# AI4Science-WestlakeU/safediffcon

Hardware: AMD Instinct MI355X
Metric: sampled control trajectories/sec (1000-step DDPM) (higher is better)
Workload: dtype f32; 1 GPU; C4: 2D smoke Unet3D_with_Conv3D dim=64 (1,2,4) state (B,32,7,64,64), B=64 per GPU, guided 1000-step DDPM, conformal quantile on; batch_per_gpu=64, global_batch=64, step=U-Net + guidance + posterior update of the whole batch, one hipGraph replay, parallelism=batch-sharded x1, no data-path collective, conv_precision=fp32

## Files before the change

include/sdc.h:

```cpp
#ifndef SDC_H
#define SDC_H

#include <stddef.h>
#include <stdint.h>

#ifdef __cplusplus
extern "C" {
#endif

#define SDC_OK 0
#define SDC_EINVAL (-1)
#define SDC_EALIGN (-2)
#define SDC_EHIP (-3)
#define SDC_ENULL (-4)

int sdc_version(void);
int sdc_last_error(char* buf, size_t cap);

typedef struct SdcConvDesc {
    int32_t B, Cin0, Cin1, Cout;
    int32_t iD, iH, iW;
    int32_t oD, oH, oW;
    int32_t kD, kH, kW;
    int32_t sD, sH, sW;
// ... 33 lines not shown
int sdc_gn_pointwise_out(const float* h, const float* stats, const float* gamma, const float* beta, const float* residual,
                         const float* w, const float* bias, float* y, int B, int C, int G, int Cout, int64_t S, int64_t plane,
                         int64_t ys0, int64_t ys1, int64_t ys2, void* stream);

int sdc_chan_norm(const float* x, const float* g, const float* residual, float* y, int B, int C, int64_t S,
                  int mode, float eps, void* stream);

int sdc_linattn(const float* qkv, float* ctx, float* out, int outer, int inner, int heads, int64_t n,
                int64_t q_so, int64_t q_sc, int64_t q_si, int64_t o_so, int64_t o_sc, int64_t o_si, void* stream);

size_t sdc_linattn_block_bytes(int outer, int inner, int C, int64_t n);
int sdc_linattn_block(const float* x, const float* g_pre, const float* wqkv, const float* wo, const float* bo,
                      const float* g_post, float* work, float* y, int outer, int inner, int C, int64_t n,
                      int64_t so, int64_t sc, int64_t si, int pre_mode, int post_mode, float eps, void* stream);
int sdc_linattn_block_gn(const float* x_raw, const float* gn_stats, const float* gn_gamma, const float* gn_beta, int gn_G,
                         const float* gn_residual, const float* g_pre, const float* wqkv, const float* wo, const float* bo,
                         const float* g_post, float* work, float* y, int outer, int inner, int C, int64_t n,
                         int64_t so, int64_t sc, int64_t si, int pre_mode, int post_mode, float eps, void* stream);
int sdc_linattn_block_sel(const float* x, const float* g_pre, const float* wqkv, const float* wo, const float* bo,
                          const float* g_post, float* work, float* y, int outer, int inner, int C, int64_t n,
                          int64_t so, int64_t sc, int64_t si, int pre_mode, int post_mode, float eps, int impl, void* stream);
int sdc_linattn_block_gn_sel(const float* x_raw, const float* gn_stats, const float* gn_gamma, const float* gn_beta, int gn_G,
                             const float* gn_residual, const float* g_pre, const float* wqkv, const float* wo, const float* bo,
                             const float* g_post, float* work, float* y, int outer, int inner, int C, int64_t n,
                             int64_t so, int64_t sc, int64_t si, int pre_mode, int post_mode, float eps, int impl, void* stream);
int sdc_linattn_block_x3_ok(int C, int64_t n);

size_t sdc_pack_linattn_f16_bytes(int C);
int sdc_pack_linattn_f16(const float* wqkv, const float* wo, int C, void* dst, void* stream);
size_t sdc_linattn_block_f16_bytes(int outer, int inner, int C, int64_t n);
int sdc_linattn_block_f16(const float* x, const float* g_pre, const float* wqkv, const float* wo, const void* wpk, const float* bo,
                          const float* g_post, void* work, float* y, int outer, int inner, int C, int64_t n,
                          int64_t so, int64_t sc, int64_t si, int pre_mode, int post_mode, float eps, void* stream);
int sdc_linattn_block_gn_f16(const float* x_raw, const float* gn_stats, const float* gn_gamma, const float* gn_beta, int gn_G,
                             const float* gn_residual, const float* g_pre, const float* wqkv, const float* wo, const void* wpk,
                             const float* bo, const float* g_post, void* work, float* y, int outer, int inner, int C, int64_t n,
                             int64_t so, int64_t sc, int64_t si, int pre_mode, int post_mode, float eps, void* stream);
int sdc_linattn_block_f16_ok(int C, int64_t n);

int sdc_tattn_block(const float* x, const float* g_pre, const float* wqkv, const float* wo, const float* rot,
                    const float* bias, float* y, int outer, int inner, int C, int ntok, int64_t so, int64_t sc,
                    int64_t st, float eps, void* stream);

size_t sdc_pack_tattn_f16_bytes(void);
int sdc_pack_tattn_f16(const float* wqkv, const float* wo, void* dst, void* stream);
int sdc_tattn_block_f16(const float* x, const float* g_pre, const void* wpk, const float* rot, const float* bias, float* y,
                        int outer, int inner, int C, int ntok, int64_t so, int64_t sc, int64_t st, float eps, void* stream);

size_t sdc_pack_tattn_x3_bytes(void);
int sdc_pack_tattn_x3(const float* wqkv, const float* wo, void* dst, void* stream);
int sdc_tattn_block_x3(const float* x, const float* g_pre, const void* wpk, const float* rot, const float* bias, float* y,
                       int outer, int inner, int C, int ntok, int64_t so, int64_t sc, int64_t st, float eps, void* stream);
int sdc_tattn_block_x3_ok(int C, int ntok, int inner);

int sdc_attn(const float* qkv, float* out, const float* rot, const float* bias, int outer, int inner, int heads,
             int ntok, int64_t q_so, int64_t q_sc, int64_t q_si, int64_t q_st,
             int64_t o_so, int64_t o_sc, int64_t o_si, int64_t o_st, void* stream);

int sdc_act(const float* x, float* y, int64_t n, int kind, void* stream);

#define SDC_MODEL_BURGERS 0
#define SDC_MODEL_TOKAMAK 1
#define SDC_MODEL_SMOKE 2

typedef struct SdcStepDesc {
    int32_t model;
    int32_t B;
    int32_t d0, d1, d2, d3;
    int32_t guide;
    int32_t clip;
    int32_t impose;
    int32_t cond_idx;
    int32_t pad_zero;
    int32_t use_max;
    int32_t has_wgt;
    int32_t skip_draws;
    int32_t ddim;
    uint64_t seed;
} SdcStepDesc;

int sdc_guide_reduce(const SdcStepDesc* d, const float* x, const float* eps, const float* coef, const int32_t* t_dev,
                     const float* gpar, float* gscal, void* stream);
int sdc_step_update(const SdcStepDesc* d, const float* x, const float* eps, const float* gext, const float* coef,
                    const int32_t* t_dev, const int32_t* draw_dev, const float* noise, int64_t noise_stride,
                    const float* gpar, const float* gscal, const float* target, const float* c0, const float* c1,
                    const float* c2, float* xout, float* x0out, void* stream);
int sdc_impose(const SdcStepDesc* d, float* x, const float* c0, const float* c1, const float* c2, void* stream);
int sdc_randn(float* x, int64_t n, uint64_t seed, const int32_t* draw_dev, void* stream);
int sdc_advance(int32_t* t_dev, int dt, int32_t* draw_dev, int ddraw, void* stream);

int sdc_advance_table(int32_t* idx_dev, int32_t* t_dev, const int32_t* ttab, int32_t* draw_dev, int ddraw, void* stream);

int sdc_conformal_score(const SdcStepDesc* d, const float* pred, const float* truth, const float* target,
                        const float* gpar, float* score, float* weight, void* stream);

int sdc_burgers_rollout(const float* u0, const float* f, float* traj, int N, int s, int Nt, int steps, int record_every,
                        float dt, float coef_transport, float d0, float d1, float d2, void* stream);


typedef struct SdcWgradDesc {
    int32_t B, M, N;
    int32_t oD, oH, oW;
    int32_t iD, iH, iW;
    int32_t kD, kH, kW;
    int32_t sD, sH, sW;
    int32_t pD, pH, pW;
// ... 187 lines not shown
```

safediffcon_amd/_lib.py:

```python
import ctypes as C
import os

_HERE = os.path.dirname(os.path.abspath(__file__))
LIB_PATH = os.path.join(_HERE, "libsdc_hip.so")

SDC_MODEL_BURGERS, SDC_MODEL_TOKAMAK, SDC_MODEL_SMOKE = 0, 1, 2

_f32p = C.c_void_p
_i32p = C.c_void_p
_stream = C.c_void_p
_i64 = C.c_int64


class SdcConvDesc(C.Structure):
    _fields_ = [(n, C.c_int32) for n in (
        "B", "Cin0", "Cin1", "Cout", "iD", "iH", "iW", "oD", "oH", "oW", "kD", "kH", "kW", "sD", "sH", "sW",
        "pD", "pH", "pW", "uD", "uH", "uW", "up_mode", "precision")] + [
        ("x0s", C.c_int64 * 5), ("x1s", C.c_int64 * 5), ("ys", C.c_int64 * 5), ("rs", C.c_int64 * 5)]


class SdcStepDesc(C.Structure):
    _fields_ = [(n, C.c_int32) for n in (
        "model", "B", "d0", "d1", "d2", "d3", "guide", "clip", "impose", "cond_idx", "pad_zero", "use_max",
        "has_wgt", "skip_draws", "ddim")] + [("_pad", C.c_int32), ("seed", C.c_uint64)]
# ... 36 lines not shown
                ("low_action", C.c_double * 9), ("high_action", C.c_double * 9), ("year_in", C.c_double)]


SIGNATURES = {
    "sdc_version": (C.c_int, []),
    "sdc_last_error": (C.c_int, [C.c_char_p, C.c_size_t]),
    "sdc_conv": (C.c_int, [C.POINTER(SdcConvDesc), _f32p, _f32p, _f32p, _f32p, _f32p, _f32p, _stream]),
    "sdc_conv_describe": (C.c_int, [C.POINTER(SdcConvDesc), C.c_char_p, C.c_size_t, C.POINTER(C.c_double)]),
    "sdc_conv_gnparts": (C.c_int, [C.POINTER(SdcConvDesc), C.c_int]),
    "sdc_conv_gn": (C.c_int, [C.POINTER(SdcConvDesc), _f32p, _f32p, _f32p, _f32p, _f32p, _f32p, C.c_void_p, C.c_int, _stream]),
    "sdc_gn_finalize": (C.c_int, [C.c_void_p, _f32p, C.c_int, C.c_int, C.c_int, _i64, C.c_float, _stream]),
    "sdc_gn_stats": (C.c_int, [_f32p, _f32p, C.c_int, C.c_int, C.c_int, _i64, C.c_float, _stream]),
    "sdc_gn_stats_bytes": (C.c_size_t, [C.c_int, C.c_int]),
    "sdc_gn_apply": (C.c_int, [_f32p, _f32p, _f32p, _f32p, _f32p, _i32p, _i64, _i64, _i64, _f32p, _f32p,
                               C.c_int, C.c_int, C.c_int, _i64, _stream]),
    "sdc_gn_fused_ok": (C.c_int, [C.c_int, C.c_int, C.c_int, _i64]),
    "sdc_gn_fused": (C.c_int, [_f32p, _f32p, _f32p, _f32p, _i32p, _i64, _i64, _i64, _f32p, _f32p, C.c_int, C.c_int, C.c_int, _i64,
                               C.c_float, _stream]),
    "sdc_gn_pointwise_out": (C.c_int, [_f32p, _f32p, _f32p, _f32p, _f32p, _f32p, _f32p, _f32p, C.c_int, C.c_int, C.c_int, C.c_int, _i64,
                                       _i64, _i64, _i64, _i64, _stream]),
    "sdc_chan_norm": (C.c_int, [_f32p, _f32p, _f32p, _f32p, C.c_int, C.c_int, _i64, C.c_int, C.c_float, _stream]),
    "sdc_linattn": (C.c_int, [_f32p, _f32p, _f32p, C.c_int, C.c_int, C.c_int, _i64, _i64, _i64, _i64, _i64, _i64,
                              _i64, _stream]),
    "sdc_linattn_block_bytes": (C.c_size_t, [C.c_int, C.c_int, C.c_int, _i64]),
    "sdc_linattn_block": (C.c_int, [_f32p, _f32p, _f32p, _f32p, _f32p, _f32p, _f32p, _f32p, C.c_int, C.c_int, C.c_int, _i64,
                                    _i64, _i64, _i64, C.c_int, C.c_int, C.c_float, _stream]),
    "sdc_linattn_block_gn": (C.c_int, [_f32p, _f32p, _f32p, _f32p, C.c_int, _f32p, _f32p, _f32p, _f32p, _f32p, _f32p, _f32p, _f32p,
                                       C.c_int, C.c_int, C.c_int, _i64, _i64, _i64, _i64, C.c_int, C.c_int, C.c_float, _stream]),
    "sdc_linattn_block_sel": (C.c_int, [_f32p, _f32p, _f32p, _f32p, _f32p, _f32p, _f32p, _f32p, C.c_int, C.c_int, C.c_int, _i64,
                                        _i64, _i64, _i64, C.c_int, C.c_int, C.c_float, C.c_int, _stream]),
    "sdc_linattn_block_gn_sel": (C.c_int, [_f32p, _f32p, _f32p, _f32p, C.c_int, _f32p, _f32p, _f32p, _f32p, _f32p, _f32p, _f32p, _f32p,
                                           C.c_int, C.c_int, C.c_int, _i64, _i64, _i64, _i64, C.c_int, C.c_int, C.c_float, C.c_int, _stream]),
    "sdc_linattn_block_x3_ok": (C.c_int, [C.c_int, _i64]),
    "sdc_pack_linattn_f16_bytes": (C.c_size_t, [C.c_int]),
    "sdc_pack_linattn_f16": (C.c_int, [_f32p, _f32p, C.c_int, C.c_void_p, _stream]),
    "sdc_linattn_block_f16_bytes": (C.c_size_t, [C.c_int, C.c_int, C.c_int, _i64]),
    "sdc_linattn_block_f16": (C.c_int, [_f32p, _f32p, _f32p, _f32p, C.c_void_p, _f32p, _f32p, C.c_void_p, _f32p, C.c_int, C.c_int,
                                        C.c_int, _i64, _i64, _i64, _i64, C.c_int, C.c_int, C.c_float, _stream]),
    "sdc_linattn_block_gn_f16": (C.c_int, [_f32p, _f32p, _f32p, _f32p, C.c_int, _f32p, _f32p, _f32p, _f32p, C.c_void_p, _f32p, _f32p,
                                           C.c_void_p, _f32p, C.c_int, C.c_int, C.c_int, _i64, _i64, _i64, _i64, C.c_int, C.c_int,
                                           C.c_float, _stream]),
    "sdc_linattn_block_f16_ok": (C.c_int, [C.c_int, _i64]),
    "sdc_tattn_block": (C.c_int, [_f32p, _f32p, _f32p, _f32p, _f32p, _f32p, _f32p, C.c_int, C.c_int, C.c_int, C.c_int,
                                  _i64, _i64, _i64, C.c_float, _stream]),
    "sdc_pack_tattn_f16_bytes": (C.c_size_t, []),
    "sdc_pack_tattn_f16": (C.c_int, [_f32p, _f32p, C.c_void_p, _stream]),
    "sdc_tattn_block_f16": (C.c_int, [_f32p, _f32p, C.c_void_p, _f32p, _f32p, _f32p, C.c_int, C.c_int, C.c_int, C.c_int,
                                      _i64, _i64, _i64, C.c_float, _stream]),
    "sdc_pack_tattn_x3_bytes": (C.c_size_t, []),
    "sdc_pack_tattn_x3": (C.c_int, [_f32p, _f32p, C.c_void_p, _stream]),
    "sdc_tattn_block_x3": (C.c_int, [_f32p, _f32p, C.c_void_p, _f32p, _f32p, _f32p, C.c_int, C.c_int, C.c_int, C.c_int,
                                     _i64, _i64, _i64, C.c_float, _stream]),
    "sdc_tattn_block_x3_ok": (C.c_int, [C.c_int, C.c_int, C.c_int]),
    "sdc_attn": (C.c_int, [_f32p, _f32p, _f32p, _f32p, C.c_int, C.c_int, C.c_int, C.c_int, _i64, _i64, _i64, _i64,
                           _i64, _i64, _i64, _i64, _stream]),
    "sdc_act": (C.c_int, [_f32p, _f32p, _i64, C.c_int, _stream]),
    "sdc_guide_reduce": (C.c_int, [C.POINTER(SdcStepDesc), _f32p, _f32p, _f32p, _i32p, _f32p, _f32p, _stream]),
    "sdc_step_update": (C.c_int, [C.POINTER(SdcStepDesc), _f32p, _f32p, _f32p, _f32p, _i32p, _i32p, _f32p, _i64,
                                  _f32p, _f32p, _f32p, _f32p, _f32p, _f32p, _f32p, _f32p, _stream]),
    "sdc_impose": (C.c_int, [C.POINTER(SdcStepDesc), _f32p, _f32p, _f32p, _f32p, _stream]),
    "sdc_randn": (C.c_int, [_f32p, _i64, C.c_uint64, _i32p, _stream]),
    "sdc_advance": (C.c_int, [_i32p, C.c_int, _i32p, C.c_int, _stream]),
    "sdc_advance_table": (C.c_int, [_i32p, _i32p, _i32p, _i32p, C.c_int, _stream]),
    "sdc_conformal_score": (C.c_int, [C.POINTER(SdcStepDesc), _f32p, _f32p, _f32p, _f32p, _f32p, _f32p, _stream]),
    "sdc_burgers_rollout": (C.c_int, [_f32p, _f32p, _f32p, C.c_int, C.c_int, C.c_int, C.c_int, C.c_int, C.c_float, C.c_float,
                                      C.c_float, C.c_float, C.c_float, _stream]),
    "sdc_conv_wgrad_bytes": (C.c_size_t, [C.POINTER(SdcWgradDesc)]),
    "sdc_conv_wgrad": (C.c_int, [C.POINTER(SdcWgradDesc), _f32p, _f32p, _f32p, _f32p, C.c_void_p, C.c_size_t, _stream]),
    "sdc_f16_grad_exponent": (C.c_int, [_f32p, C.c_int, C.c_int, C.c_int, C.c_int, C.c_int, C.c_void_p, C.c_void_p, _stream]),
    "sdc_conv_dgrad_f16": (C.c_int, [C.POINTER(SdcConvDesc), _f32p, _f32p, C.c_void_p, _f32p, _stream]),
    "sdc_conv_stem_f16_ok": (C.c_int, [C.POINTER(SdcConvDesc)]),
    "sdc_pack_stem_f16_bytes": (C.c_size_t, [C.c_int, C.c_int, C.c_int, C.c_int, C.c_int]),
    "sdc_pack_stem_f16": (C.c_int, [_f32p, C.c_void_p, C.c_int, C.c_int, C.c_int, C.c_int, C.c_int, _stream]),
    "sdc_conv_stem_f16": (C.c_int, [C.POINTER(SdcConvDesc), _f32p, C.c_void_p, _f32p, _f32p, _stream]),
    "sdc_conv_stem_x3_ok": (C.c_int, [C.POINTER(SdcConvDesc)]),
    "sdc_pack_stem_x3_bytes": (C.c_size_t, [C.c_int, C.c_int, C.c_int, C.c_int, C.c_int]),
    "sdc_pack_stem_x3": (C.c_int, [_f32p, C.c_void_p, C.c_int, C.c_int, C.c_int, C.c_int, C.c_int, _stream]),
    "sdc_conv_stem_x3": (C.c_int, [C.POINTER(SdcConvDesc), _f32p, C.c_void_p, _f32p, _f32p, _stream]),
    "sdc_conv_gemm_x3_ok": (C.c_int, [C.POINTER(SdcConvDesc)]),
    "sdc_pack_gemm_x3_bytes": (C.c_size_t, [C.c_int, C.c_int, C.c_int, C.c_int]),
    "sdc_pack_gemm_x3": (C.c_int, [_f32p, C.c_void_p, C.c_int, C.c_int, C.c_int, C.c_int, _stream]),
    "sdc_conv_gemm_x3": (C.c_int, [C.POINTER(SdcConvDesc), _f32p, C.c_void_p, _f32p, _f32p, _stream]),
    "sdc_conv_pw_x3_ok": (C.c_int, [C.POINTER(SdcConvDesc)]),
    "sdc_conv_pw_x3": (C.c_int, [C.POINTER(SdcConvDesc), _f32p, _f32p, _f32p, _f32p, _f32p, _f32p, _stream]),
    "sdc_conv_wino3_x3_ok": (C.c_int, [C.POINTER(SdcConvDesc)]),
    "sdc_pack_wino3_x3_bytes": (C.c_size_t, [C.c_int, C.c_int]),
    "sdc_pack_wino3_x3": (C.c_int, [_f32p, C.c_void_p, C.c_int, C.c_int, _stream]),
    "sdc_conv_wino3_x3": (C.c_int, [C.POINTER(SdcConvDesc), _f32p, _f32p, C.c_void_p, _f32p, _f32p, C.c_void_p, C.c_int, _stream]),
    "sdc_conv_wgrad_f16_bytes": (C.c_size_t, [C.POINTER(SdcWgradDesc)]),
    "sdc_conv_wgrad_f16": (C.c_int, [C.POINTER(SdcWgradDesc), _f32p, _f32p, C.c_void_p, _f32p, _f32p, C.c_void_p, C.c_size_t, _stream]),
    "sdc_conv_wgrad_describe": (C.c_int, [C.POINTER(SdcWgradDesc), C.c_char_p, C.c_size_t]),
    "sdc_gn_silu_bwd_floats": (C.c_size_t, [C.c_int, C.c_int, C.c_int, _i64]),
    "sdc_gn_silu_bwd": (C.c_int, [_f32p, _f32p, _f32p, _f32p, _f32p, _f32p, _i64, _f32p, _f32p, _f32p, _f32p, _f32p,
                                  C.c_int, C.c_int, C.c_int, _i64, _stream]),
    "sdc_chan_norm_bwd_parts": (C.c_size_t, [C.c_int, _i64]),
    "sdc_chan_norm_bwd_bytes": (C.c_size_t, [C.c_int, C.c_int, _i64]),
    "sdc_chan_norm_bwd": (C.c_int, [_f32p, _f32p, _f32p, _f32p, _f32p, C.c_int, C.c_int, _i64, C.c_int, C.c_float, _stream]),
    "sdc_pack_conv_weight_floats": (C.c_size_t, [C.c_int, C.c_int, C.c_int, C.c_int, C.c_int, C.c_int]),
    "sdc_pack_conv_weight": (C.c_int, [_f32p, _f32p, C.c_int, C.c_int, C.c_int, C.c_int, C.c_int, C.c_int, C.c_int, _stream]),
    "sdc_pack_batch_plan": (C.c_int, [C.POINTER(SdcPackItem), C.c_int, C.POINTER(C.c_int), C.POINTER(C.c_int)]),
    "sdc_pack_batch_run": (C.c_int, [C.c_void_p, C.c_int, C.c_int, C.c_int, _stream]),
    "sdc_tattn_block_bwd_bytes": (C.c_size_t, [C.c_int, C.c_int]),
    "sdc_tattn_block_bwd": (C.c_int, [_f32p, _f32p, _f32p, _f32p, _f32p, _f32p, _f32p, _f32p, _f32p, _f32p, _f32p, _f32p, C.c_void_p,
                                      C.c_int, C.c_int, C.c_int, C.c_int, _i64, _i64, _i64, C.c_float, _stream]),
    "sdc_linattn_block_bwd_bytes": (C.c_size_t, [C.c_int, C.c_int, C.c_int, _i64]),
    "sdc_linattn_block_bwd": (C.c_int, [_f32p, _f32p, _f32p, _f32p, _f32p, _f32p, _f32p, _f32p, _f32p, _f32p, _f32p, C.c_void_p,
# ... 74 lines not shown
```

safediffcon_amd/csrc/sdc_tablock_x3.hip:

```cpp
#define TA_WEIGHT_ARGS const __bf16* wpk;
#include "sdc_tablock_tile.h"
#include "sdc_split3.h"

namespace {

constexpr int XF = 68;
constexpr int XPP = 32 * XF + 8;
constexpr int WQKV_E = 3 * 4 * 64 * 8;
constexpr int HEAD_E = WQKV_E + 2 * 2 * 64 * 8;
constexpr int WPK_E = 4 * 3 * HEAD_E;
constexpr int WBUF_B = 3 * HEAD_E * 2;
constexpr int REGB_B = NS * XPP * 4;
static_assert(WBUF_B <= REGB_B && 32 * XP * 4 <= REGB_B, "region B holds a head's weights and a y half");
static_assert(WBUF_B % (16 * NT) == 0, "whole 16-byte words per thread");

__device__ __forceinline__ ta2 ta_rot(ta2 x, ta2 cs) {
#pragma clang fp contract(off)
    const float t0 = x.x * cs.x, t1 = x.y * cs.x;
    return ta2{__builtin_fmaf(-x.y, cs.y, t0), __builtin_fmaf(x.x, cs.y, t1)};
}

__global__ __launch_bounds__(NT) void ta_block_x3_kernel(const TaArgs a) {
    extern __shared__ __attribute__((aligned(16))) unsigned char smem_x3[];
    unsigned char* const wA = smem_x3;
    unsigned char* const rB = smem_x3 + WBUF_B;
    float* const xim = reinterpret_cast<float*>(rB);
    float* const ys = reinterpret_cast<float*>(rB);
    float* const biasT = reinterpret_cast<float*>(rB + REGB_B);
    float* const rotcs = biasT + 4 * 32 * 33;
    float* const red = rotcs + 2 * 32 * 16;

    const int tid = threadIdx.x, lane = tid & 63, wave = tid >> 6, l31 = lane & 31, lh = lane >> 5;
    const TaWalk wk = ta_walk(a.nblk);
    const int per = wk.per, first = wk.first, stride = wk.stride;

    const int tok = tid & 255, half = tid >> 8, pw = tok & 7, f = tok >> 3;
    const uint32_t toff = (uint32_t)(((int64_t)f * a.st + pw) * 4);

    u32x4 wreg[6];
    auto fetch_head = [&](int head) {
        const u32x4* src = reinterpret_cast<const u32x4*>(a.wpk) + head * (WBUF_B / 16) + tid;
#pragma unroll
        for (int i = 0; i < 6; ++i) wreg[i] = src[i * NT];
    };
    auto park_head = [&](unsigned char* wb) {
        u32x4* dst = reinterpret_cast<u32x4*>(wb) + tid;
#pragma unroll
        for (int i = 0; i < 6; ++i) dst[i * NT] = wreg[i];
    };

    float v[32];
    if (first < per) {
        const float* xt = a.x + ta_tile_ptr(a, wk, first) + (int64_t)(half * 32) * a.sc;
#pragma unroll
        for (int c = 0; c < 32; ++c) v[c] = ldu(uni(xt + (int64_t)c * a.sc), toff);
    }
    {
        fetch_head(0);
#pragma unroll
        for (int i = 0; i < 8; ++i) {
            const int e = tid + i * NT, h = e >> 10, q = (e >> 5) & 31, kk = e & 31;
            biasT[(h * 32 + kk) * 33 + q] = (a.bias ? a.bias[e] : 0.0f) * 5.65685424949238f;
        }
        const float2 rr = a.rot ? *reinterpret_cast<const float2*>(a.rot + tid * 2) : make_float2(1.0f, 0.0f);
        *reinterpret_cast<float2*>(rotcs + (((tid & 15) * 32) + (tid >> 4)) * 2) = rr;
        park_head(wA);
    }
    const int hw = wave;

    for (int li = first; li < per; li += stride) {
        const int64_t tp = ta_tile_ptr(a, wk, li);
        const bool more = li + stride < per;
        {
            float sm = 0.f;
#pragma unroll
            for (int c = 0; c < 32; ++c) sm += v[c];
            red[half * 256 + tok] = sm;
            __syncthreads();
            const float mean = (red[tok] + red[256 + tok]) * (1.0f / C);
            float q = 0.f;
#pragma unroll
            for (int c = 0; c < 32; ++c) { v[c] -= mean; q += v[c] * v[c]; }
            red[512 + half * 256 + tok] = q;
            __syncthreads();
            const float rstd = rsqrtf((red[512 + tok] + red[768 + tok]) * (1.0f / C) + a.eps);
            nfloat4* xo = reinterpret_cast<nfloat4*>(xim + pw * XPP + f * XF + half * 32);
#pragma unroll
            for (int c4 = 0; c4 < 8; ++c4) {
                nfloat4 o;
#pragma unroll
                for (int j = 0; j < 4; ++j) o[j] = v[c4 * 4 + j] * rstd * a.g[half * 32 + c4 * 4 + j];
                xo[c4] = o;
            }
        }
        __syncthreads();
        bf16x8 xf[3][4];
        {
            const float* xr = xim + hw * XPP + l31 * XF + 8 * lh;
#pragma unroll
            for (int s = 0; s < 4; ++s) {
                const nfloat4 lo = *reinterpret_cast<const nfloat4*>(xr + 16 * s), hi = *reinterpret_cast<const nfloat4*>(xr + 16 * s + 4);
                const float xv[8] = {lo[0], lo[1], lo[2], lo[3], hi[0], hi[1], hi[2], hi[3]};
                split3x8(xv, xf[0][s], xf[1][s], xf[2][s]);
            }
        }
        f32x16 yacc[2];
#pragma unroll
        for (int i = 0; i < 2; ++i)
#pragma unroll
            for (int r = 0; r < 16; ++r) yacc[i][r] = 0.f;
#pragma unroll 1
        for (int head = 0; head < 4; ++head) {
            const unsigned char* const wh = (head & 1) ? rB : wA;
            unsigned char* const wn = (head & 1) ? wA : rB;
            __syncthreads();
            const bool next = head < 3 || more;
            if (next) fetch_head((head + 1) & 3);
            const bf16x8* wf = reinterpret_cast<const bf16x8*>(wh) + lane;
            f32x16 q, k, vt;
#pragma unroll
            for (int r = 0; r < 16; ++r) { q[r] = 0.f; k[r] = 0.f; vt[r] = 0.f; }
#pragma unroll
            for (int t = 0; t < 6; ++t)
#pragma unroll
                for (int s = 0; s < 4; ++s) {
                    const bf16x8* wp = wf + X3_PA[t] * (HEAD_E / 8);
                    q = __builtin_amdgcn_mfma_f32_32x32x16_bf16(wp[(0 * 4 + s) * 64], xf[X3_PB[t]][s], q, 0, 0, 0);
                    k = __builtin_amdgcn_mfma_f32_32x32x16_bf16(wp[(1 * 4 + s) * 64], xf[X3_PB[t]][s], k, 0, 0, 0);
                    vt = __builtin_amdgcn_mfma_f32_32x32x16_bf16(xf[X3_PB[t]][s], wp[(2 * 4 + s) * 64], vt, 0, 0, 0);
                    if (s == 3) __builtin_amdgcn_sched_barrier(0);
                }
            if (next) park_head(wn);
#pragma unroll
            for (int r = 0; r < 16; r += 2) {
                const int m = crow(r, lh) >> 1;
                const ta2 cs = *reinterpret_cast<const ta2*>(rotcs + (m * 32 + l31) * 2);
                ta2 q2 = {q[r], q[r + 1]}, k2 = {k[r], k[r + 1]};
                q2 = ta_rot(q2, cs);
                k2 = ta_rot(k2, cs);
                q[r] = q2.x; q[r + 1] = q2.y;
                k[r] = k2.x; k[r + 1] = k2.y;
            }
            f32x16 acc;
#pragma unroll
            for (int r = 0; r < 16; ++r) acc[r] = biasT[(head * 32 + crow(r, lh)) * 33 + l31];
#pragma unroll
            for (int r = 0; r < 16; ++r) acc = __builtin_amdgcn_mfma_f32_32x32x2f32(k[r], q[r], acc, 0, 0, 0);
            float mx = -INFINITY;
#pragma unroll
            for (int r = 0; r < 16; ++r) mx = fmaxf(mx, acc[r]);
            mx = fmaxf(mx, __shfl_xor(mx, 32, 64));
            const float SL = 0.17677669529663687f * 1.4426950408889634f;
            const float nmx = -mx * SL;
            float sum = 0.f;
#pragma unroll
            for (int r = 0; r < 16; ++r) { acc[r] = __builtin_amdgcn_exp2f(fmaf(acc[r], SL, nmx)); sum += acc[r]; }
            sum += __shfl_xor(sum, 32, 64);
            const float inv = 1.0f / sum;
#pragma unroll
            for (int r = 0; r < 16; ++r) acc[r] *= inv;
            f32x16 oacc;
#pragma unroll
            for (int r = 0; r < 16; ++r) oacc[r] = 0.f;
#pragma unroll
            for (int r = 0; r < 16; ++r) oacc = __builtin_amdgcn_mfma_f32_32x32x2f32(vt[r], acc[r], oacc, 0, 0, 0);
            bf16x8 of[3][2];
#pragma unroll
            for (int s = 0; s < 2; ++s) {
                float ov[8];
#pragma unroll
                for (int j = 0; j < 8; ++j) ov[j] = oacc[8 * s + j];
                split3x8(ov, of[0][s], of[1][s], of[2][s]);
            }
            const bf16x8* wof = wf + WQKV_E / 8;
#pragma unroll
            for (int t = 0; t < 6; ++t)
#pragma unroll
                for (int s = 0; s < 2; ++s) {
                    const bf16x8* wp = wof + X3_PA[t] * (HEAD_E / 8);
                    yacc[0] = __builtin_amdgcn_mfma_f32_32x32x16_bf16(wp[(0 * 2 + s) * 64], of[X3_PB[t]][s], yacc[0], 0, 0, 0);
                    yacc[1] = __builtin_amdgcn_mfma_f32_32x32x16_bf16(wp[(1 * 2 + s) * 64], of[X3_PB[t]][s], yacc[1], 0, 0, 0);
                }
        }
        {
            const float* xt = a.x + ta_tile_ptr(a, wk, more ? li + stride : li) + (int64_t)(half * 32) * a.sc;
#pragma unroll
            for (int c = 0; c < 32; ++c) v[c] = ldu(uni(xt + (int64_t)c * a.sc), toff);
        }
#pragma unroll
        for (int i = 0; i < 2; ++i) {
            float xr[16];
            const int64_t ch0 = (int64_t)(i * 32 + half * 16) * a.sc;
            const float* xt = a.x + tp + ch0;
#pragma unroll
            for (int c = 0; c < 16; ++c) xr[c] = ldu(uni(xt + (int64_t)c * a.sc), toff);
            __syncthreads();
#pragma unroll
            for (int r = 0; r < 16; ++r) ys[crow(r, lh) * XP + hw * 33 + l31] = yacc[i][r];
            __syncthreads();
            const float* yt = a.y + tp + ch0;
#pragma unroll
            for (int c = 0; c < 16; ++c) stu(uni(yt + (int64_t)c * a.sc), toff, ys[(half * 16 + c) * XP + pw * 33 + f] + xr[c]);
        }
        __syncthreads();
    }
}

__global__ __launch_bounds__(256) void pack_tattn_x3_kernel(const float* __restrict__ wqkv, const float* __restrict__ wo,
                                                            __bf16* __restrict__ dst) {
    const int g = blockIdx.x * 256 + threadIdx.x;
    if (g >= 4 * HEAD_E) return;
    const int head = g / HEAD_E, e = g - head * HEAD_E;
    const int j = e & 7, lane = (e >> 3) & 63, l31 = lane & 31, lh = lane >> 5;
    float wv;
    if (e < WQKV_E) {
        const int s = (e >> 9) & 3, mat = e >> 11;
        wv = wqkv[(mat * 128 + head * 32 + l31) * C + 16 * s + 8 * lh + j];
    } else {
        const int e2 = e - WQKV_E, s = (e2 >> 9) & 1, i = (e2 >> 10) & 1;
        wv = wo[(32 * i + l31) * 128 + head * 32 + crow(8 * s + j, lh)];
    }
    __bf16 ph, pm, pl;
    split3(wv, ph, pm, pl);
    __bf16* d = dst + (int64_t)head * 3 * HEAD_E + e;
    d[0] = ph; d[HEAD_E] = pm; d[2 * HEAD_E] = pl;
}

bool sdc_tattn_x3_faster(int Cc, int ntok, int inner) {
    return Cc == 64 && ntok == 32 && inner == 4096;
}

}

extern "C" int sdc_tattn_block_x3_ok(int Cc, int ntok, int inner) { return sdc_tattn_x3_faster(Cc, ntok, inner) ? 1 : 0; }

extern "C" size_t sdc_pack_tattn_x3_bytes(void) { return (size_t)WPK_E * sizeof(__bf16); }

extern "C" int sdc_pack_tattn_x3(const float* wqkv, const float* wo, void* dst, void* stream) {
    SDC_REQUIRE(wqkv && wo && dst, SDC_ENULL, "sdc_pack_tattn_x3: null pointer");
    SDC_REQUIRE(reinterpret_cast<uintptr_t>(dst) % 16 == 0, SDC_EALIGN, "sdc_pack_tattn_x3: dst must be 16-byte aligned");
    hipLaunchKernelGGL(pack_tattn_x3_kernel, dim3(4 * HEAD_E / 256), dim3(256), 0, sdc::as_stream(stream), wqkv, wo,
                       reinterpret_cast<__bf16*>(dst));
    return sdc::check_launch("sdc_pack_tattn_x3");
}

extern "C" int sdc_tattn_block_x3(const float* x, const float* g_pre, const void* wpk, const float* rot, const float* bias, float* y,
                                  int outer, int inner, int Cc, int ntok, int64_t so, int64_t sc, int64_t st, float eps, void* stream) {
    SDC_REQUIRE(wpk, SDC_ENULL, "sdc_tattn_block_x3: null pointer");
    TaArgs a;
    if (const int rc = ta_check_args("sdc_tattn_block_x3", x, g_pre, rot, bias, y, outer, inner, Cc, ntok, so, sc, st, eps, a)) return rc;
    a.wpk = reinterpret_cast<const __bf16*>(wpk);
    SDC_REQUIRE(reinterpret_cast<uintptr_t>(wpk) % 16 == 0, SDC_EALIGN, "sdc_tattn_block_x3: the weight buffer must be 16-byte aligned");
    SDC_REQUIRE(!rot || reinterpret_cast<uintptr_t>(rot) % 8 == 0, SDC_EINVAL, "sdc_tattn_block_x3: rot must be 8-byte aligned");
    const size_t ldsb = (size_t)WBUF_B + REGB_B + sizeof(float) * (size_t)(4 * 32 * 33 + 2 * 32 * 16 + 1024);
    static std::atomic<uint64_t> attr{0};
    SDC_LDS_OPTIN(attr, ta_block_x3_kernel, 160 * 1024, "sdc_tattn_block_x3");
    unsigned grid = 0;
    if (const int rc = sdc::ta_grid("sdc_tattn_block_x3", a.nblk, &grid)) return rc;
    hipLaunchKernelGGL(ta_block_x3_kernel, dim3(grid), dim3(NT), ldsb, sdc::as_stream(stream), a);
    return sdc::check_launch("sdc_tattn_block_x3");
}
```

Measured before the change: 0.3096 trajectories/s.

## Restructure temporal-attention x3 kernel with buffer loads, residual reuse, optional skewed waves

Reworks the fused temporal-attention block kernel into a templated tile routine. The default path now keeps the pre-norm input values in registers for the residual add and writes the full 64-channel y image in one LDS pass, using raw buffer loads and stores instead of reloading x. This is meant to remove a second global read of the residual and one pair of barriers per tile. It also adds an opt-in skewed variant in which half the waves lag by one head, to overlap MFMA with softmax and other VALU work, plus compile-gated debug/ablation variants. Holding x in registers raises register pressure, and the skewed variant needs extra LDS.

```diff
diff --git a/include/sdc.h b/include/sdc.h
--- a/include/sdc.h
+++ b/include/sdc.h
@@ -109,6 +109,9 @@
 int sdc_tattn_block_x3(const float* x, const float* g_pre, const void* wpk, const float* rot, const float* bias, float* y,
                        int outer, int inner, int C, int ntok, int64_t so, int64_t sc, int64_t st, float eps, void* stream);
 int sdc_tattn_block_x3_ok(int C, int ntok, int inner);
+int sdc_tattn_block_x3_sel(const float* x, const float* g_pre, const void* wpk, const float* rot, const float* bias, float* y,
+                           int outer, int inner, int C, int ntok, int64_t so, int64_t sc, int64_t st, float eps, int impl, void* stream);
+int sdc_tattn_block_x3_impl(int C, int ntok, int inner);
 
 int sdc_attn(const float* qkv, float* out, const float* rot, const float* bias, int outer, int inner, int heads,
              int ntok, int64_t q_so, int64_t q_sc, int64_t q_si, int64_t q_st,
diff --git a/safediffcon_amd/_lib.py b/safediffcon_amd/_lib.py
--- a/safediffcon_amd/_lib.py
+++ b/safediffcon_amd/_lib.py
@@ -112,6 +112,9 @@
     "sdc_tattn_block_x3": (C.c_int, [_f32p, _f32p, C.c_void_p, _f32p, _f32p, _f32p, C.c_int, C.c_int, C.c_int, C.c_int,
                                      _i64, _i64, _i64, C.c_float, _stream]),
     "sdc_tattn_block_x3_ok": (C.c_int, [C.c_int, C.c_int, C.c_int]),
+    "sdc_tattn_block_x3_sel": (C.c_int, [_f32p, _f32p, C.c_void_p, _f32p, _f32p, _f32p, C.c_int, C.c_int, C.c_int, C.c_int,
+                                         _i64, _i64, _i64, C.c_float, C.c_int, _stream]),
+    "sdc_tattn_block_x3_impl": (C.c_int, [C.c_int, C.c_int, C.c_int]),
     "sdc_attn": (C.c_int, [_f32p, _f32p, _f32p, _f32p, C.c_int, C.c_int, C.c_int, C.c_int, _i64, _i64, _i64, _i64,
                            _i64, _i64, _i64, _i64, _stream]),
     "sdc_act": (C.c_int, [_f32p, _f32p, _i64, C.c_int, _stream]),
diff --git a/safediffcon_amd/csrc/sdc_tablock_x3.hip b/safediffcon_amd/csrc/sdc_tablock_x3.hip
--- a/safediffcon_amd/csrc/sdc_tablock_x3.hip
+++ b/safediffcon_amd/csrc/sdc_tablock_x3.hip
@@ -11,7 +11,7 @@
 constexpr int WPK_E = 4 * 3 * HEAD_E;
 constexpr int WBUF_B = 3 * HEAD_E * 2;
 constexpr int REGB_B = NS * XPP * 4;
-static_assert(WBUF_B <= REGB_B && 32 * XP * 4 <= REGB_B, "region B holds a head's weights and a y half");
+static_assert(WBUF_B <= REGB_B && 64 * XP * 4 <= REGB_B, "region B holds a head's weights and the y image");
 static_assert(WBUF_B % (16 * NT) == 0, "whole 16-byte words per thread");
 
 __device__ __forceinline__ ta2 ta_rot(ta2 x, ta2 cs) {
@@ -20,7 +20,44 @@
     return ta2{__builtin_fmaf(-x.y, cs.y, t0), __builtin_fmaf(x.x, cs.y, t1)};
 }
 
-__global__ __launch_bounds__(NT) void ta_block_x3_kernel(const TaArgs a) {
+__device__ __forceinline__ __amdgpu_buffer_rsrc_t ta_buf(const float* p) {
+    return __builtin_amdgcn_make_buffer_rsrc(const_cast<float*>(p), 0, 0xffffffff, 0x00020000);
+}
+__device__ __forceinline__ float ldb(__amdgpu_buffer_rsrc_t r, uint32_t tok_off, uint32_t chan_off) {
+    return __builtin_bit_cast(float, __builtin_amdgcn_raw_buffer_load_b32(r, tok_off, chan_off, 0));
+}
+__device__ __forceinline__ void stb(__amdgpu_buffer_rsrc_t r, uint32_t tok_off, uint32_t chan_off, float v) {
+    __builtin_amdgcn_raw_buffer_store_b32(__builtin_bit_cast(uint32_t, v), r, tok_off, chan_off, 0);
+}
+
+constexpr int XD_LN = 1;
+constexpr int XD_EXIT = 2;
+constexpr int XD_SPLIT = 4;
+constexpr int XD_WFETCH = 8;
+constexpr int XD_FRAG = 16;
+constexpr int XD_BAR = 32;
+constexpr int XD_VALU = 64;
+[[maybe_unused]] constexpr int XD_MFMA_ONLY = 127;
+constexpr int XD_STORE = 128;
+constexpr int XD_RES = 256;
+constexpr int XD_XNEXT = 512;
+
+template <int DBG>
+__device__ __forceinline__ void ta_split3x8(const float* v, bf16x8& h, bf16x8& m, bf16x8& l) {
+    if constexpr (DBG & XD_SPLIT) {
+        const nfloat4 lo = {v[0], v[1], v[2], v[3]}, hi = {v[4], v[5], v[6], v[7]};
+        h = __builtin_bit_cast(bf16x8, lo); m = __builtin_bit_cast(bf16x8, hi); l = h;
+    } else {
+        split3x8(v, h, m, l);
+    }
+}
+
+constexpr int WOS_P = 2 * 2 * 64;
+constexpr int WOS_B = 3 * WOS_P * 16;
+constexpr int TAB_B = 4 * (4 * 32 * 33 + 2 * 32 * 16 + 1024);
+
+template <bool SKEW, int EXIT, int DBG>
+__device__ __forceinline__ void ta_x3_tiles(const TaArgs& a) {
     extern __shared__ __attribute__((aligned(16))) unsigned char smem_x3[];
     unsigned char* const wA = smem_x3;
     unsigned char* const rB = smem_x3 + WBUF_B;
@@ -29,8 +66,10 @@
     float* const biasT = reinterpret_cast<float*>(rB + REGB_B);
     float* const rotcs = biasT + 4 * 32 * 33;
     float* const red = rotcs + 2 * 32 * 16;
+    unsigned char* const wE = rB + REGB_B + TAB_B;
 
     const int tid = threadIdx.x, lane = tid & 63, wave = tid >> 6, l31 = lane & 31, lh = lane >> 5;
+    const bool lag = SKEW && __builtin_amdgcn_readfirstlane(tid) >= NT / 2;
     const TaWalk wk = ta_walk(a.nblk);
     const int per = wk.per, first = wk.first, stride = wk.stride;
 
@@ -38,25 +77,33 @@
     const uint32_t toff = (uint32_t)(((int64_t)f * a.st + pw) * 4);
 
     u32x4 wreg[6];
-    auto fetch_head = [&](int head) {
+    auto fetch_head = [&](int head, int wo) {
+        if constexpr (DBG & XD_WFETCH) return;
         const u32x4* src = reinterpret_cast<const u32x4*>(a.wpk) + head * (WBUF_B / 16) + tid;
 #pragma unroll
-        for (int i = 0; i < 6; ++i) wreg[i] = src[i * NT];
+        for (int i = 0; i < 6; ++i)
+            if (!SKEW || wo == 0 || (((i & 1) && lag) == (wo > 0))) wreg[i] = src[i * NT];
     };
-    auto park_head = [&](unsigned char* wb) {
+    auto park_head = [&](unsigned char* wb, int wo) {
+        if constexpr (DBG & XD_WFETCH) return;
         u32x4* dst = reinterpret_cast<u32x4*>(wb) + tid;
 #pragma unroll
-        for (int i = 0; i < 6; ++i) dst[i * NT] = wreg[i];
+        for (int i = 0; i < 6; ++i)
+            if (!SKEW || wo == 0 || (((i & 1) && lag) == (wo > 0))) dst[i * NT] = wreg[i];
     };
+    auto wo_base = [&](int head) -> unsigned char* { return head == 2 ? wE : ((head == 1) ? rB : wA) + WQKV_E * 2; };
+    auto wo_pitch = [&](int head) -> int { return head == 2 ? WOS_P : HEAD_E / 8; };
 
     float v[32];
+    const uint32_t sc4 = (uint32_t)a.sc * 4u;
+    const uint32_t hoff = (uint32_t)__builtin_amdgcn_readfirstlane(half) * 32u * sc4;
     if (first < per) {
-        const float* xt = a.x + ta_tile_ptr(a, wk, first) + (int64_t)(half * 32) * a.sc;
-#pragma unroll
-        for (int c = 0; c < 32; ++c) v[c] = ldu(uni(xt + (int64_t)c * a.sc), toff);
+        const __amdgpu_buffer_rsrc_t xb = ta_buf(a.x + ta_tile_ptr(a, wk, first));
+#pragma unroll
+        for (int c = 0; c < 32; ++c) v[c] = ldb(xb, toff, hoff + (uint32_t)c * sc4);
     }
     {
-        fetch_head(0);
+        fetch_head(0, 0);
 #pragma unroll
         for (int i = 0; i < 8; ++i) {
             const int e = tid + i * NT, h = e >> 10, q = (e >> 5) & 31, kk = e & 31;
@@ -64,15 +111,23 @@
         }
         const float2 rr = a.rot ? *reinterpret_cast<const float2*>(a.rot + tid * 2) : make_float2(1.0f, 0.0f);
         *reinterpret_cast<float2*>(rotcs + (((tid & 15) * 32) + (tid >> 4)) * 2) = rr;
-        park_head(wA);
+        park_head(wA, 0);
     }
     const int hw = wave;
 
     for (int li = first; li < per; li += stride) {
         const int64_t tp = ta_tile_ptr(a, wk, li);
         const bool more = li + stride < per;
-        {
+        float xr1[EXIT >= 1 ? 32 : 1];
+        if constexpr (DBG & XD_LN) {
+#pragma unroll
+            for (int c = 0; c < 32; ++c) asm volatile("" ::"v"(v[c]));
+        } else {
             float sm = 0.f;
+            if constexpr (EXIT == 2) {
+#pragma unroll
+                for (int c = 0; c < 32; ++c) xr1[c] = v[c];
+            }
 #pragma unroll
             for (int c = 0; c < 32; ++c) sm += v[c];
             red[half * 256 + tok] = sm;
@@ -101,7 +156,7 @@
             for (int s = 0; s < 4; ++s) {
                 const nfloat4 lo = *reinterpret_cast<const nfloat4*>(xr + 16 * s), hi = *reinterpret_cast<const nfloat4*>(xr + 16 * s + 4);
                 const float xv[8] = {lo[0], lo[1], lo[2], lo[3], hi[0], hi[1], hi[2], hi[3]};
-                split3x8(xv, xf[0][s], xf[1][s], xf[2][s]);
+                ta_split3x8<DBG>(xv, xf[0][s], xf[1][s], xf[2][s]);
             }
         }
         f32x16 yacc[2];
@@ -109,15 +164,10 @@
         for (int i = 0; i < 2; ++i)
 #pragma unroll
             for (int r = 0; r < 16; ++r) yacc[i][r] = 0.f;
-#pragma unroll 1
-        for (int head = 0; head < 4; ++head) {
-            const unsigned char* const wh = (head & 1) ? rB : wA;
-            unsigned char* const wn = (head & 1) ? wA : rB;
-            __syncthreads();
-            const bool next = head < 3 || more;
-            if (next) fetch_head((head + 1) & 3);
+        f32x16 q, k, vt;
+        auto front = [&](const unsigned char* wh, int nh, bool next) {
+            if (next) fetch_head(nh, (SKEW && nh == 0) ? -1 : 0);
             const bf16x8* wf = reinterpret_cast<const bf16x8*>(wh) + lane;
-            f32x16 q, k, vt;
 #pragma unroll
             for (int r = 0; r < 16; ++r) { q[r] = 0.f; k[r] = 0.f; vt[r] = 0.f; }
 #pragma unroll
@@ -125,12 +175,30 @@
 #pragma unroll
                 for (int s = 0; s < 4; ++s) {
                     const bf16x8* wp = wf + X3_PA[t] * (HEAD_E / 8);
-                    q = __builtin_amdgcn_mfma_f32_32x32x16_bf16(wp[(0 * 4 + s) * 64], xf[X3_PB[t]][s], q, 0, 0, 0);
-                    k = __builtin_amdgcn_mfma_f32_32x32x16_bf16(wp[(1 * 4 + s) * 64], xf[X3_PB[t]][s], k, 0, 0, 0);
-                    vt = __builtin_amdgcn_mfma_f32_32x32x16_bf16(xf[X3_PB[t]][s], wp[(2 * 4 + s) * 64], vt, 0, 0, 0);
+                    const bf16x8 wq = (DBG & XD_FRAG) ? xf[X3_PA[t]][s] : wp[(0 * 4 + s) * 64];
+                    const bf16x8 wkk = (DBG & XD_FRAG) ? xf[X3_PA[t]][s ^ 1] : wp[(1 * 4 + s) * 64];
+                    const bf16x8 wv = (DBG & XD_FRAG) ? xf[X3_PA[t]][s ^ 2] : wp[(2 * 4 + s) * 64];
+                    q = __builtin_amdgcn_mfma_f32_32x32x16_bf16(wq, xf[X3_PB[t]][s], q, 0, 0, 0);
+                    k = __builtin_amdgcn_mfma_f32_32x32x16_bf16(wkk, xf[X3_PB[t]][s], k, 0, 0, 0);
+                    vt = __builtin_amdgcn_mfma_f32_32x32x16_bf16(xf[X3_PB[t]][s], wv, vt, 0, 0, 0);
                     if (s == 3) __builtin_amdgcn_sched_barrier(0);
                 }
-            if (next) park_head(wn);
+            if (next) {
+                if (!SKEW || nh == 1) {
+                    park_head((nh & 1) ? rB : wA, 0);
+                } else {
+                    park_head((nh & 1) ? rB : wA, -1);
+                    if (nh != 0 && lag) {
+                        if constexpr (!(DBG & XD_WFETCH)) {
+                            u32x4* dst = reinterpret_cast<u32x4*>(wo_base(nh)) + (tid - NT / 2);
+                            const int pitch = wo_pitch(nh);
+#pragma unroll
+                            for (int p = 0; p < 3; ++p) dst[p * pitch] = wreg[2 * p + 1];
+                        }
+                    }
+                }
+            }
+            if constexpr (DBG & XD_VALU) return;
 #pragma unroll
             for (int r = 0; r < 16; r += 2) {
                 const int m = crow(r, lh) >> 1;
@@ -141,24 +209,28 @@
                 q[r] = q2.x; q[r + 1] = q2.y;
                 k[r] = k2.x; k[r + 1] = k2.y;
             }
+        };
+        auto tail = [&](int head, const bf16x8* wof, int wop) {
             f32x16 acc;
 #pragma unroll
-            for (int r = 0; r < 16; ++r) acc[r] = biasT[(head * 32 + crow(r, lh)) * 33 + l31];
+            for (int r = 0; r < 16; ++r) acc[r] = (DBG & XD_VALU) ? 0.f : biasT[(head * 32 + crow(r, lh)) * 33 + l31];
 #pragma unroll
             for (int r = 0; r < 16; ++r) acc = __builtin_amdgcn_mfma_f32_32x32x2f32(k[r], q[r], acc, 0, 0, 0);
-            float mx = -INFINITY;
-#pragma unroll
-            for (int r = 0; r < 16; ++r) mx = fmaxf(mx, acc[r]);
-            mx = fmaxf(mx, __shfl_xor(mx, 32, 64));
-            const float SL = 0.17677669529663687f * 1.4426950408889634f;
-            const float nmx = -mx * SL;
-            float sum = 0.f;
-#pragma unroll
-            for (int r = 0; r < 16; ++r) { acc[r] = __builtin_amdgcn_exp2f(fmaf(acc[r], SL, nmx)); sum += acc[r]; }
-            sum += __shfl_xor(sum, 32, 64);
-            const float inv = 1.0f / sum;
-#pragma unroll
-            for (int r = 0; r < 16; ++r) acc[r] *= inv;
+            if constexpr (!(DBG & XD_VALU)) {
+                float mx = -INFINITY;
+#pragma unroll
+                for (int r = 0; r < 16; ++r) mx = fmaxf(mx, acc[r]);
+                mx = fmaxf(mx, __shfl_xor(mx, 32, 64));
+                const float SL = 0.17677669529663687f * 1.4426950408889634f;
+                const float nmx = -mx * SL;
+                float sum = 0.f;
+#pragma unroll
+                for (int r = 0; r < 16; ++r) { acc[r] = __builtin_amdgcn_exp2f(fmaf(acc[r], SL, nmx)); sum += acc[r]; }
+                sum += __shfl_xor(sum, 32, 64);
+                const float inv = 1.0f / sum;
+#pragma unroll
+                for (int r = 0; r < 16; ++r) acc[r] *= inv;
+            }
             f32x16 oacc;
 #pragma unroll
             for (int r = 0; r < 16; ++r) oacc[r] = 0.f;
@@ -170,41 +242,101 @@
                 float ov[8];
 #pragma unroll
                 for (int j = 0; j < 8; ++j) ov[j] = oacc[8 * s + j];
-                split3x8(ov, of[0][s], of[1][s], of[2][s]);
-            }
-            const bf16x8* wof = wf + WQKV_E / 8;
+                ta_split3x8<DBG>(ov, of[0][s], of[1][s], of[2][s]);
+            }
 #pragma unroll
             for (int t = 0; t < 6; ++t)
 #pragma unroll
                 for (int s = 0; s < 2; ++s) {
-                    const bf16x8* wp = wof + X3_PA[t] * (HEAD_E / 8);
-                    yacc[0] = __builtin_amdgcn_mfma_f32_32x32x16_bf16(wp[(0 * 2 + s) * 64], of[X3_PB[t]][s], yacc[0], 0, 0, 0);
-                    yacc[1] = __builtin_amdgcn_mfma_f32_32x32x16_bf16(wp[(1 * 2 + s) * 64], of[X3_PB[t]][s], yacc[1], 0, 0, 0);
+                    const bf16x8* wp = wof + X3_PA[t] * wop;
+                    const bf16x8 w0 = (DBG & XD_FRAG) ? xf[X3_PA[t]][s] : wp[(0 * 2 + s) * 64];
+                    const bf16x8 w1 = (DBG & XD_FRAG) ? xf[X3_PA[t]][s + 2] : wp[(1 * 2 + s) * 64];
+                    yacc[0] = __builtin_amdgcn_mfma_f32_32x32x16_bf16(w0, of[X3_PB[t]][s], yacc[0], 0, 0, 0);
+                    yacc[1] = __builtin_amdgcn_mfma_f32_32x32x16_bf16(w1, of[X3_PB[t]][s], yacc[1], 0, 0, 0);
                 }
-        }
-        {
-            const float* xt = a.x + ta_tile_ptr(a, wk, more ? li + stride : li) + (int64_t)(half * 32) * a.sc;
-#pragma unroll
-            for (int c = 0; c < 32; ++c) v[c] = ldu(uni(xt + (int64_t)c * a.sc), toff);
-        }
-#pragma unroll
-        for (int i = 0; i < 2; ++i) {
-            float xr[16];
-            const int64_t ch0 = (int64_t)(i * 32 + half * 16) * a.sc;
-            const float* xt = a.x + tp + ch0;
-#pragma unroll
-            for (int c = 0; c < 16; ++c) xr[c] = ldu(uni(xt + (int64_t)c * a.sc), toff);
+        };
+#pragma unroll 1
+        for (int head = 0; head < 4; ++head) {
+            const unsigned char* const wh = (head & 1) ? rB : wA;
+            if constexpr (!(DBG & XD_BAR))
+                __syncthreads();
+            const bool next = head < 3 || more;
+            if constexpr (SKEW) {
+                if (lag && head > 0) tail(head - 1, reinterpret_cast<const bf16x8*>(wo_base(head - 1)) + lane, wo_pitch(head - 1));
+                __builtin_amdgcn_sched_barrier(0);
+                front(wh, (head + 1) & 3, next);
+                if (!lag) tail(head, reinterpret_cast<const bf16x8*>(wo_base(head)) + lane, wo_pitch(head));
+            } else {
+                front(wh, (head + 1) & 3, next);
+                tail(head, reinterpret_cast<const bf16x8*>(wh) + lane + WQKV_E / 8, HEAD_E / 8);
+            }
+        }
+        if constexpr (SKEW) {
+            if (lag) tail(3, reinterpret_cast<const bf16x8*>(wo_base(3)) + lane, wo_pitch(3));
+            if (more) fetch_head(0, +1);
+        }
+        const __amdgpu_buffer_rsrc_t xb = ta_buf(a.x + tp), yb = ta_buf(a.y + tp);
+        if constexpr (EXIT == 1 && !(DBG & XD_EXIT)) {
+#pragma unroll
+            for (int c = 0; c < 32; ++c) xr1[c] = ldb(xb, toff, hoff + (uint32_t)c * sc4);
+        }
+        if constexpr (!(DBG & XD_XNEXT)) {
+            const __amdgpu_buffer_rsrc_t xn = ta_buf(a.x + ta_tile_ptr(a, wk, more ? li + stride : li));
+#pragma unroll
+            for (int c = 0; c < 32; ++c) v[c] = ldb(xn, toff, hoff + (uint32_t)c * sc4);
+        }
+        if constexpr (DBG & XD_EXIT) {
+#pragma unroll
+            for (int i = 0; i < 2; ++i)
+#pragma unroll
+                for (int r = 0; r < 16; ++r) asm volatile("" ::"v"(yacc[i][r]));
             __syncthreads();
-#pragma unroll
-            for (int r = 0; r < 16; ++r) ys[crow(r, lh) * XP + hw * 33 + l31] = yacc[i][r];
+        } else if constexpr (EXIT >= 1) {
             __syncthreads();
-            const float* yt = a.y + tp + ch0;
-#pragma unroll
-            for (int c = 0; c < 16; ++c) stu(uni(yt + (int64_t)c * a.sc), toff, ys[(half * 16 + c) * XP + pw * 33 + f] + xr[c]);
+            if constexpr (SKEW)
+                if (more) park_head(wA, +1);
+#pragma unroll
+            for (int i = 0; i < 2; ++i)
+#pragma unroll
+                for (int r = 0; r < 16; ++r) ys[(i * 32 + crow(r, lh)) * XP + hw * 33 + l31] = yacc[i][r];
+            __syncthreads();
+#pragma unroll
+            for (int c = 0; c < 32; ++c) stb(yb, toff, hoff + (uint32_t)c * sc4, ys[(half * 32 + c) * XP + pw * 33 + f] + xr1[c]);
+        } else {
+#pragma unroll
+            for (int i = 0; i < 2; ++i) {
+                float xr[16];
+                const uint32_t ch0 = (uint32_t)i * 32u * sc4 + (hoff >> 1);
+#pragma unroll
+                for (int c = 0; c < 16; ++c) xr[c] = (DBG & XD_RES) ? 0.f : ldb(xb, toff, ch0 + (uint32_t)c * sc4);
+                __syncthreads();
+                if constexpr (SKEW)
+                    if (i == 1 && more) park_head(wA, +1);
+#pragma unroll
+                for (int r = 0; r < 16; ++r) ys[crow(r, lh) * XP + hw * 33 + l31] = yacc[i][r];
+                __syncthreads();
+#pragma unroll
+                for (int c = 0; c < 16; ++c) {
+                    const float yv = ys[(half * 16 + c) * XP + pw * 33 + f] + xr[c];
+                    if constexpr (DBG & XD_STORE) asm volatile("" ::"v"(yv));
+                    else stb(yb, toff, ch0 + (uint32_t)c * sc4, yv);
+                }
+            }
         }
         __syncthreads();
     }
 }
+
+__global__ __launch_bounds__(NT) void ta_block_x3_kernel(const TaArgs a) { ta_x3_tiles<false, 2, 0>(a); }
+
+__global__ __launch_bounds__(NT) void ta_block_x3s_kernel(const TaArgs a) { ta_x3_tiles<true, 1, 0>(a); }
+
+#ifdef SDC_KERNEL_EXPERIMENTS
+template <bool SKEW, int EXIT>
+__global__ __launch_bounds__(NT) void ta_block_x3_form_kernel(const TaArgs a) { ta_x3_tiles<SKEW, EXIT, 0>(a); }
+template <int DBG>
+__global__ __launch_bounds__(NT) void ta_block_x3_dbg_kernel(const TaArgs a) { ta_x3_tiles<false, 0, DBG>(a); }
+#endif
 
 __global__ __launch_bounds__(256) void pack_tattn_x3_kernel(const float* __restrict__ wqkv, const float* __restrict__ wo,
                                                             __bf16* __restrict__ dst) {
@@ -244,19 +376,78 @@
     return sdc::check_launch("sdc_pack_tattn_x3");
 }
 
+namespace {
+
+int tattn_block_x3_impl(const char* who, const float* x, const float* g_pre, const void* wpk, const float* rot, const float* bias,
+                        float* y, int outer, int inner, int Cc, int ntok, int64_t so, int64_t sc, int64_t st, float eps, int impl,
+                        void* stream) {
+    SDC_REQUIRE(wpk, SDC_ENULL, "%s: null pointer", who);
+    SDC_REQUIRE(impl == 0 || impl == 1, SDC_EINVAL, "%s: impl must be 0 or 1 (got %d)", who, impl);
+    TaArgs a;
+    if (const int rc = ta_check_args(who, x, g_pre, rot, bias, y, outer, inner, Cc, ntok, so, sc, st, eps, a)) return rc;
+    a.wpk = reinterpret_cast<const __bf16*>(wpk);
+    SDC_REQUIRE(reinterpret_cast<uintptr_t>(wpk) % 16 == 0, SDC_EALIGN, "%s: the weight buffer must be 16-byte aligned", who);
+    SDC_REQUIRE(!rot || reinterpret_cast<uintptr_t>(rot) % 8 == 0, SDC_EINVAL, "%s: rot must be 8-byte aligned", who);
+    const size_t ldsb = (size_t)WBUF_B + REGB_B + TAB_B;
+    unsigned grid = 0;
+    if (const int rc = sdc::ta_grid(who, a.nblk, &grid)) return rc;
+#define TAX3_LAUNCH(KERNEL, LDS)                                                                      \
+    do {                                                                                              \
+        static std::atomic<uint64_t> attr{0};                                                         \
+        SDC_LDS_OPTIN(attr, KERNEL, 160 * 1024, who);                                                 \
+        hipLaunchKernelGGL(KERNEL, dim3(grid), dim3(NT), LDS, sdc::as_stream(stream), a);             \
+        return sdc::check_launch(who);                                                                \
+    } while (0)
+#ifdef SDC_KERNEL_EXPERIMENTS
+    static const int form = getenv("SDC_TAX3_FORM") ? atoi(getenv("SDC_TAX3_FORM")) : -1;
+    switch (form) {
+        case 0: TAX3_LAUNCH((ta_block_x3_form_kernel<false, 0>), ldsb);
+        case 1: TAX3_LAUNCH((ta_block_x3_form_kernel<true, 0>), ldsb + WOS_B);
+        case 2: TAX3_LAUNCH((ta_block_x3_form_kernel<false, 1>), ldsb);
+        case 3: TAX3_LAUNCH((ta_block_x3_form_kernel<true, 1>), ldsb + WOS_B);
+        case 4: TAX3_LAUNCH((ta_block_x3_form_kernel<false, 2>), ldsb);
+        case 5: TAX3_LAUNCH((ta_block_x3_form_kernel<true, 2>), ldsb + WOS_B);
+        default: break;
+    }
+#endif
+    if (impl == 1) TAX3_LAUNCH(ta_block_x3s_kernel, ldsb + WOS_B);
+#ifdef SDC_KERNEL_EXPERIMENTS
+    static const int dbg = getenv("SDC_TAX3_DBG") ? atoi(getenv("SDC_TAX3_DBG")) : 0;
+    switch (dbg) {
+        case 0: break;
+        case XD_LN: TAX3_LAUNCH(ta_block_x3_dbg_kernel<XD_LN>, ldsb);
+        case XD_EXIT: TAX3_LAUNCH(ta_block_x3_dbg_kernel<XD_EXIT>, ldsb);
+        case XD_SPLIT: TAX3_LAUNCH(ta_block_x3_dbg_kernel<XD_SPLIT>, ldsb);
+        case XD_WFETCH: TAX3_LAUNCH(ta_block_x3_dbg_kernel<XD_WFETCH>, ldsb);
+        case XD_FRAG: TAX3_LAUNCH(ta_block_x3_dbg_kernel<XD_FRAG>, ldsb);
+        case XD_BAR: TAX3_LAUNCH(ta_block_x3_dbg_kernel<XD_BAR>, ldsb);
+        case XD_VALU: TAX3_LAUNCH(ta_block_x3_dbg_kernel<XD_VALU>, ldsb);
+        case XD_STORE: TAX3_LAUNCH(ta_block_x3_dbg_kernel<XD_STORE>, ldsb);
+        case XD_RES: TAX3_LAUNCH(ta_block_x3_dbg_kernel<XD_RES>, ldsb);
+        case XD_XNEXT: TAX3_LAUNCH(ta_block_x3_dbg_kernel<XD_XNEXT>, ldsb);
+        case XD_STORE | XD_RES | XD_XNEXT: TAX3_LAUNCH(ta_block_x3_dbg_kernel<XD_STORE | XD_RES | XD_XNEXT>, ldsb);
+        default: TAX3_LAUNCH(ta_block_x3_dbg_kernel<XD_MFMA_ONLY>, ldsb);
+    }
+#endif
+    TAX3_LAUNCH(ta_block_x3_kernel, ldsb);
+#undef TAX3_LAUNCH
+}
+
+}
+
+extern "C" int sdc_tattn_block_x3_impl(int Cc, int ntok, int inner) {
+    (void)Cc; (void)ntok; (void)inner;
+    return 0;
+}
+
+extern "C" int sdc_tattn_block_x3_sel(const float* x, const float* g_pre, const void* wpk, const float* rot, const float* bias, float* y,
+                                      int outer, int inner, int Cc, int ntok, int64_t so, int64_t sc, int64_t st, float eps, int impl,
+                                      void* stream) {
+    return tattn_block_x3_impl("sdc_tattn_block_x3_sel", x, g_pre, wpk, rot, bias, y, outer, inner, Cc, ntok, so, sc, st, eps, impl, stream);
+}
+
 extern "C" int sdc_tattn_block_x3(const float* x, const float* g_pre, const void* wpk, const float* rot, const float* bias, float* y,
                                   int outer, int inner, int Cc, int ntok, int64_t so, int64_t sc, int64_t st, float eps, void* stream) {
-    SDC_REQUIRE(wpk, SDC_ENULL, "sdc_tattn_block_x3: null pointer");
-    TaArgs a;
-    if (const int rc = ta_check_args("sdc_tattn_block_x3", x, g_pre, rot, bias, y, outer, inner, Cc, ntok, so, sc, st, eps, a)) return rc;
-    a.wpk = reinterpret_cast<const __bf16*>(wpk);
-    SDC_REQUIRE(reinterpret_cast<uintptr_t>(wpk) % 16 == 0, SDC_EALIGN, "sdc_tattn_block_x3: the weight buffer must be 16-byte aligned");
-    SDC_REQUIRE(!rot || reinterpret_cast<uintptr_t>(rot) % 8 == 0, SDC_EINVAL, "sdc_tattn_block_x3: rot must be 8-byte aligned");
-    const size_t ldsb = (size_t)WBUF_B + REGB_B + sizeof(float) * (size_t)(4 * 32 * 33 + 2 * 32 * 16 + 1024);
-    static std::atomic<uint64_t> attr{0};
-    SDC_LDS_OPTIN(attr, ta_block_x3_kernel, 160 * 1024, "sdc_tattn_block_x3");
-    unsigned grid = 0;
-    if (const int rc = sdc::ta_grid("sdc_tattn_block_x3", a.nblk, &grid)) return rc;
-    hipLaunchKernelGGL(ta_block_x3_kernel, dim3(grid), dim3(NT), ldsb, sdc::as_stream(stream), a);
-    return sdc::check_launch("sdc_tattn_block_x3");
-}
+    return tattn_block_x3_impl("sdc_tattn_block_x3", x, g_pre, wpk, rot, bias, y, outer, inner, Cc, ntok, so, sc, st, eps,
+                               sdc_tattn_block_x3_impl(Cc, ntok, inner), stream);
+}
```

Measured after the change: 0.3128 trajectories/s (median of 6 runs). 1.0% higher.
